# Grid2op/grid2op

Hardware: AMD Instinct MI355X
Metric: env steps/sec (batched DoNothing) (higher is better)
Workload: dtype f64; 1 GPU; l2rpn_case14_sandbox AC Newton-Raphson DoNothing env.step, batch=4096 lanes per GPU; env=l2rpn_case14_sandbox, lanes_per_gpu=4096, total_lanes=4096, env_steps_per_launch=16, observations=every env step -> HBM, cascade=False, kernels=grid-specialised at run time (gpf_jit_enable), parallelism=static lane shards x1, no collective

## Files before the change

### grid2op_amd/csrc/gridpf_sparse.hpp

```cpp
#pragma once
#include <type_traits>
#include "gridpf_common.hpp"

namespace gpf {

struct StatOff {
  int n_dbl, n_int;
  int n_int_hot;
  int br_y, br_bdc, sub_vn_kv, shunt_fact, gen_min_q, gen_max_q;
  int line_vn, load_vn, gen_vn, sto_vn, shunt_vn;
  int line_ka;
  int gen_qmin_tot, gen_qmax_tot;
  int gen_cnt;
  int dc_inv;
  int line_or_pos, line_ex_pos, line_or_sub, line_ex_sub, br_slot, gen_pos, gen_sub, gen_slack, load_pos, load_sub, sto_pos,
      sto_sub, shunt_sub, pair_rc, up, prog;
  int pos_line;
};
#define GPF_STATOFF_INTS(X) X(n_dbl) X(n_int) X(n_int_hot) X(br_y) X(br_bdc) X(sub_vn_kv) X(shunt_fact) X(gen_min_q) X(gen_max_q) X(line_vn) X(load_vn) \
  X(gen_vn) X(sto_vn) X(shunt_vn) X(line_ka) X(gen_qmin_tot) X(gen_qmax_tot) X(gen_cnt) X(dc_inv) X(line_or_pos) X(line_ex_pos) X(line_or_sub) \
  X(line_ex_sub) X(br_slot) X(gen_pos) X(gen_sub) X(gen_slack) X(load_pos) X(load_sub) X(sto_pos) X(sto_sub) X(shunt_sub) X(pair_rc) X(up) X(prog) X(pos_line)
static_assert(sizeof(StatOff) == sizeof(int) * (0 GPF_STATOFF_INTS(GPF_COUNT_FIELD)), "GPF_STATOFF_INTS must list every field of StatOff");
template <class T, bool IN_LDS>
struct SP {
// ... 1109 lines not shown
    if (PROG_LDS) return scalar_lu_flat<GW, true, false>(FL, sv.prog.p, c.A, c.A, tid, dbg);
    return scalar_lu_flat<GW, true, false>(FL, gptr(flat_g), c.A, c.A, tid, dbg);
  };
  if (!warm && !fuse_dc) {
#ifdef GPF_TIMING
    bool ok = dc_inv ? true : (NB == 1) ? lu_dc(&stamps.v[20])
                                        : lu_ac(&stamps.v[20]);
#else
    bool ok = dc_inv ? true : (NB == 1) ? lu_dc(nullptr) : lu_ac(nullptr);
#endif
    for (int i = tid; i < nbus; i += GW) {
      double th;
      if (dc_inv) {
        auto row_times_rhs = [&](const auto tab) -> double {
          double t0 = 0.0, t1 = 0.0;
          for (int k0 = 0; k0 < nbus; k0 += MVC) {
            double a_[MVC], r_[MVC];
#pragma unroll
            for (int q = 0; q < MVC; ++q) {
              const int k = k0 + q < nbus ? k0 + q : nbus - 1;
              a_[q] = tab[k * nbus + i];
              r_[q] = *rhsT(k);
            }
#pragma unroll
            for (int q = 0; q < MVC; q += 2) {
              if (k0 + q < nbus) t0 = fma(a_[q], r_[q], t0);
              if (k0 + q + 1 < nbus) t1 = fma(a_[q + 1], r_[q + 1], t1);
            }
          }
          return t0 + t1;
        };
        th = S.so.dc_inv >= 0 ? row_times_rhs(sv.dc_inv) : row_times_rhs(sv.dc_inv_g);
      } else if (NB == 1) {
        const double d = dc_kept ? c.Adc[i] : c.A[(size_t)i * 2];
        if (!(fabs(d) > 1e-300) || !(fabs(d) < 1e300)) ok = false;
        th = *rhsT(i) * fast_rcp(d);
      } else th = *rhsT(i);
      const int bt = c.btype[i];
      c.va[i] = (bt == BT_PQ || bt == BT_PV) ? th : 0.0;
      if (bt != BT_OFF && !(fabs(th) < 1e300)) ok = false;
    }
    if (NB == 1 && ctl.dcf && !dc_skip)
      for (int q = tid; q < S.nslot; q += GW) c.Adc[q] = c.A[(size_t)q * 2];
    GPF_LSYNC();
    if (WPI == 1 && dc_inv && G::block_any_u(ts.dc_out >= 0)) {
      const int lo_ = ts.dc_out >= 0 ? ts.dc_out : 0;
      const int f_ = sv.line_or_sub[lo_], t_ = sv.line_ex_sub[lo_];
      const double bl = ts.dc_out >= 0 ? sv.br_bdc[lo_] : 0.0;
      const bool f_ref = c.btype[f_] == BT_REF, t_ref = c.btype[t_] == BT_REF;
      const double dth = c.va[f_] - c.va[t_];
      const double xff = f_ref ? 0.0 : dcinv(f_ * nbus + f_), xtt = t_ref ? 0.0 : dcinv(t_ * nbus + t_);
      const double xft = (f_ref || t_ref) ? 0.0 : dcinv(t_ * nbus + f_);
      const double den = 1.0 - bl * (xff - 2.0 * xft + xtt);
      if (!(fabs(den) > 1e-12)) ok = false;
      const double kk = bl * dth / den;
      for (int i = tid; i < nbus; i += GW) {
        const int bt = c.btype[i];
        const double u_ = (f_ref ? 0.0 : dcinv(f_ * nbus + i)) - (t_ref ? 0.0 : dcinv(t_ * nbus + i));
        if (bt == BT_PQ || bt == BT_PV) c.va[i] += u_ * kk;
      }
      GPF_LSYNC();
    }
    if (status == 0 && G::any(!ok)) status = 4;
    if (G::block_all_u(status != 0)) return status;
  }
  GPF_STAMPS(4);

  int it = 0;
  if (!is_dc) {
    bool converged = false;
    bool done = status != 0;
    const int n_pairs = S.nslot_y * NB * NB;
    auto t_of = [&](const double2 y, double ei, double fi, double ej, double fj, double& tr_, double& ti_) {
      const double aa = y.x * ej - y.y * fj, bb = y.x * fj + y.y * ej;
      tr_ = ei * aa + fi * bb;
      ti_ = fi * aa - ei * bb;
    };
    if (nwr) {
      const bool p_on = tid < S.n_up, b_on = tid < nbus;
      const int ib = b_on ? tid : 0;
      const unsigned w0 = p_on ? (unsigned)sv.up[2 * tid] : 0u, w1 = p_on ? (unsigned)sv.up[2 * tid + 1] : 0u;
      const int u = (int)(w0 & 0xffffu), v = (int)(w0 >> 16), suv = (int)(w1 & 0xffffu), svu = (int)(w1 >> 16);
      constexpr bool KEEP_Y = IPW > 1;
      const double2* const p_yuv = reinterpret_cast<const double2*>(c.Yb + (size_t)suv * 2);
      const double2* const p_yvu = reinterpret_cast<const double2*>(c.Yb + (size_t)svu * 2);
      const double2* const p_yd = reinterpret_cast<const double2*>(c.Yb + (size_t)ib * 2);
      const double2 yuv0 = *p_yuv, yvu0 = *p_yvu, ydiag0 = *p_yd;
      const int btu = c.btype[u], btv = c.btype[v];
      const int bt = c.btype[ib];
      const double psp0 = c.Psp[ib], qsp0 = c.Qsp[ib];
#define NWR_YUV (KEEP_Y ? yuv0 : *p_yuv)
#define NWR_YVU (KEEP_Y ? yvu0 : *p_yvu)
#define NWR_YD (KEEP_Y ? ydiag0 : *p_yd)
#define NWR_PSP (KEEP_Y ? psp0 : c.Psp[ib])
#define NWR_QSP (KEEP_Y ? qsp0 : c.Qsp[ib])
      double va, vm;
#ifdef GPF_TIMING
      asm volatile("s_waitcnt lgkmcnt(0)" ::: "memory");
      GPF_STAMPS(20);
#endif
      if (fuse_dc) {
        const int vi = fast_pre ? c.vidx[ib] : -1;
        const double vm_lds = fast_pre ? 1.0 : c.vm[ib];
        if (b_on) c.ivm[ib] = psp0 - c.Gs[ib];
        GPF_LSYNC();
        auto row_times_rhs = [&](const auto tab, const bool by_row) -> double {
          double t0 = 0.0, t1 = 0.0;
          for (int k0 = 0; k0 < nbus; k0 += MVC) {
            double a_[MVC], r_[MVC];
#pragma unroll
            for (int q = 0; q < MVC; ++q) {
              const int k = k0 + q < nbus ? k0 + q : nbus - 1;
              a_[q] = by_row ? tab[ib * nbus + k] : tab[k * nbus + ib];
              r_[q] = c.ivm[k];
            }
#pragma unroll
            for (int q = 0; q < MVC; q += 2) {
              if (k0 + q < nbus) t0 = fma(a_[q], r_[q], t0);
              if (k0 + q + 1 < nbus) t1 = fma(a_[q + 1], r_[q + 1], t1);
            }
          }
          return t0 + t1;
        };
        const double th = S.so.dc_inv >= 0 ? row_times_rhs(sv.dc_inv, STAGE == 2) : row_times_rhs(sv.dc_inv_g, false);
        const bool live = (bt == BT_PQ || bt == BT_PV);
        va = live ? th : 0.0;
        vm = (vi >= 0 && (bt == BT_PV || bt == BT_REF)) ? GPF_INJ(oo.inj_gen_vm + vi) : vm_lds;
        const bool th_bad = b_on && bt != BT_OFF && !(fabs(th) < 1e300);
        if (status == 0 && G::any(th_bad)) { status = 4; done = true; }
      } else { va = c.va[ib]; vm = c.vm[ib]; }
#ifdef GPF_TIMING
      GPF_STAMPS(21);
#endif
      const bool act = p_on && (btu != BT_OFF) && (btv != BT_OFF);
      const bool uP = (btu == BT_PQ || btu == BT_PV), uQ = (btu == BT_PQ), vP = (btv == BT_PQ || btv == BT_PV), vQ = (btv == BT_PQ);
      const bool acc_u = act && (yuv0.x != 0.0 || yuv0.y != 0.0), acc_v = act && (yvu0.x != 0.0 || yvu0.y != 0.0);
      const bool rowP = (bt == BT_PQ || bt == BT_PV), rowQ = (bt == BT_PQ);
      const bool diag_on = bt != BT_OFF && (ydiag0.x != 0.0 || ydiag0.y != 0.0);
      double* const Ad0 = bel(ib, 0, 0);
      double* const Ad1 = bel(ib, 1, 0);
      double* const b_uv0 = bel(suv, 0, 0); double* const b_uv1 = bel(suv, 1, 0);
      double* const b_vu0 = bel(svu, 0, 0); double* const b_vu1 = bel(svu, 1, 0);
      double e, f, ivm, Sr = 0.0, Si = 0.0;
      {
        double sn_, co;
        fast_sincos(va, sn_, co);
        e = vm * co; f = vm * sn_; ivm = fast_rcp(vm);
        if (b_on) { setEF(ib, e, f); c.ivm[ib] = ivm; *SreP(ib) = 0.0; *SimP(ib) = 0.0; }
      }
      for (int i = S.nslot_y * 2 + tid; i < S.nslot * 2; i += GW) { c.A[i] = 0.0; c.A[HS + i] = 0.0; }
      GPF_LSYNC();
      GPF_STAMPS(10);
      asm volatile("; GPF_NEWTON_NWR_BEGIN" ::: "memory");
      while (true) {
        if (p_on) {
          const double2 efu = EF(u), efv = EF(v);
          const double ivmu = c.ivm[u], ivmv = c.ivm[v];
          double tr_, ti_, sr_, si_;
          const double2 yuv = NWR_YUV, yvu = NWR_YVU;
          t_of(yuv, efu.x, efu.y, efv.x, efv.y, tr_, ti_);
          t_of(yvu, efv.x, efv.y, efu.x, efu.y, sr_, si_);
          *reinterpret_cast<double2*>(b_uv0) = make_double2((uP && vP) ? ti_ : 0.0, (uP && vQ) ? tr_ * ivmv : 0.0);
          *reinterpret_cast<double2*>(b_uv1) = make_double2((uQ && vP) ? -tr_ : 0.0, (uQ && vQ) ? ti_ * ivmv : 0.0);
          *reinterpret_cast<double2*>(b_vu0) = make_double2((vP && uP) ? si_ : 0.0, (vP && uQ) ? sr_ * ivmu : 0.0);
          *reinterpret_cast<double2*>(b_vu1) = make_double2((vQ && uP) ? -sr_ : 0.0, (vQ && uQ) ? si_ * ivmu : 0.0);
          if (acc_u) { atomicAdd(SreP(u), tr_); atomicAdd(SimP(u), ti_); }
          if (acc_v) { atomicAdd(SreP(v), sr_); atomicAdd(SimP(v), si_); }
        }
        GPF_LSYNC();
        if (it == 0) GPF_STAMPS(11);
        double fabs_mis = 0.0;
        bool bad = false;
        if (b_on) {
          Sr = *SreP(ib); Si = *SimP(ib);
          const double2 ydiag = NWR_YD;
          const double psp = NWR_PSP, qsp = NWR_QSP;
          double tr_, ti_;
          t_of(ydiag, e, f, e, f, tr_, ti_);
          if (diag_on) { Sr += tr_; Si += ti_; }
          const double2 r0 = make_double2(rowP ? ti_ : 0.0, (rowP && rowQ) ? tr_ * ivm : 0.0);
          const double2 r1 = make_double2((rowQ && rowP) ? -tr_ : 0.0, rowQ ? ti_ * ivm : 0.0);
          *reinterpret_cast<double2*>(Ad0) = make_double2(rowP ? r0.x - Si : 1.0, rowQ ? fma(Sr, ivm, r0.y) : r0.y);
          *reinterpret_cast<double2*>(Ad1) = make_double2(rowQ ? r1.x + Sr : r1.x, rowQ ? fma(Si, ivm, r1.y) : 1.0);
          const double mp = rowP ? (Sr - psp) : 0.0;
          const double mq = rowQ ? (Si - qsp) : 0.0;
          *rhsT(ib) = -mp; *rhsV(ib) = -mq;
          const double am = fmax(fabs(mp), fabs(mq));
          if (!(am <= 1e300)) bad = true;
          fabs_mis = am;
        }
        if (!done) {
          const unsigned fl = G::template any2<0>(!(fabs_mis < tol_pu), bad);
          if (fl & 2u) { status = 1; done = true; }
          else if (!(fl & 1u)) { converged = true; done = true; }
          else if (it >= max_iter) done = true;
          else ++it;
        }
        if (G::block_all_u(done)) break;
        GPF_LSYNC();
        if (it == 1) GPF_STAMPS(12);
#ifdef GPF_TIMING
        const bool ok = lu_ac(it == 1 ? &stamps.v[32] : nullptr);
#else
        const bool ok = lu_ac(nullptr);
#endif
        if (it == 1) GPF_STAMPS(13);
        bool fin = true, piv_ok = true;
        if (b_on) {
          double2 dx = make_double2(*rhsT(ib), *rhsV(ib));
          const double2 dA = *reinterpret_cast<const double2*>(Ad0), dB = *reinterpret_cast<const double2*>(Ad1);
          const double det = fma(dA.x, dB.y, -dA.y * dB.x);
          if (!(fabs(det) > 1e-300) || !(fabs(det) < 1e300)) piv_ok = false;
          const double rd = fast_rcp(det);
          dx = make_double2(fma(dB.y, dx.x, -dA.y * dx.y) * rd, fma(dA.x, dx.y, -dB.x * dx.x) * rd);
          if (!done && bt != BT_OFF) {
            if (!(fabs(dx.x) < 1e300) || !(fabs(dx.y) < 1e300)) fin = false;
            if (bt == BT_PQ || bt == BT_PV) va += dx.x;
            if (bt == BT_PQ) vm += dx.y;
            if (vm < 0.0) { vm = -vm; va += 3.14159265358979323846; }
            if (fabs(va) > 3.14159265358979323846) va = remainder(va, 6.28318530717958647692);
          }
          double sn_, co;
          fast_sincos(va, sn_, co);
          e = vm * co; f = vm * sn_; ivm = fast_rcp(vm);
          setEF(ib, e, f);
          c.ivm[ib] = ivm;
          *SreP(ib) = 0.0;
          *SimP(ib) = 0.0;
        }
        for (int i = S.nslot_y * 2 + tid; i < S.nslot * 2; i += GW) { c.A[i] = 0.0; c.A[HS + i] = 0.0; }
        GPF_LSYNC();
        if (!done && G::template any2<1>(!ok || !piv_ok, !fin) != 0u) { status = 4; done = true; }
        if (it == 1) GPF_STAMPS(14);
        asm volatile("; GPF_NEWTON_NWR_BACKEDGE" ::: "memory");
      }
      if (b_on) { *SreP(ib) = Sr; *SimP(ib) = Si; c.va[ib] = va; c.vm[ib] = vm; }
#undef NWR_YUV
#undef NWR_YVU
#undef NWR_YD
#undef NWR_PSP
#undef NWR_QSP
    } else {
      for (int i = tid; i < nbus; i += GW) {
        const double va = c.va[i], vmi = c.vm[i];
        double sn_, co;
        fast_sincos(va, sn_, co);
        setEF(i, vmi * co, vmi * sn_);
        if (NB == 1) c.ivm[i] = fast_rcp(vmi);
        *SreP(i) = 0.0;
        *SimP(i) = 0.0;
        if (WPI > 1) { *rhsT(i) = 0.0; *rhsV(i) = 0.0; }
      }
      if (BS == 2) { for (int i = S.nslot_y * 2 + tid; i < S.nslot * 2; i += GW) { c.A[i] = 0.0; c.A[HS + i] = 0.0; } }
      else for (int i = S.nslot_y * B2 + tid; i < S.nslot_lu * B2; i += GW) c.A[i] = 0.0;
      GPF_LSYNC();
      GPF_STAMPS(10);
      unsigned rc_first = 0, rc_first1 = 0;
      if (STAGE == 0 && !YR) {
        if (NB == 1) { if (tid < S.n_up) { rc_first = (unsigned)sv.up[2 * tid]; rc_first1 = (unsigned)sv.up[2 * tid + 1]; } }
        else if (tid < n_pairs) rc_first = (unsigned)sv.pair_rc[tid / (NB * NB)];
      }
      while (true) {
        if (NB == 1) {
          auto upair_item = [&](const unsigned w0, const unsigned w1, const double2 yuv, const double2 yvu) {
            const int u = (int)(w0 & 0xffffu), v = (int)(w0 >> 16), suv = (int)(w1 & 0xffffu), svu = (int)(w1 >> 16);
            const int btu = c.btype[u], btv = c.btype[v];
            const double2 efu = EF(u), efv = EF(v);
            const double eu = efu.x, fu = efu.y, ivmu = c.ivm[u], ev = efv.x, fv = efv.y, ivmv = c.ivm[v];
            double tr_, ti_, sr_, si_;
            t_of(yuv, eu, fu, ev, fv, tr_, ti_);
            t_of(yvu, ev, fv, eu, fu, sr_, si_);
            const bool act = (btu != BT_OFF) && (btv != BT_OFF);
            const bool uP = (btu == BT_PQ || btu == BT_PV), uQ = (btu == BT_PQ), vP = (btv == BT_PQ || btv == BT_PV), vQ = (btv == BT_PQ);
            *reinterpret_cast<double2*>(bel(suv, 0, 0)) = make_double2((uP && vP) ? ti_ : 0.0, (uP && vQ) ? tr_ * ivmv : 0.0);
            *reinterpret_cast<double2*>(bel(suv, 1, 0)) = make_double2((uQ && vP) ? -tr_ : 0.0, (uQ && vQ) ? ti_ * ivmv : 0.0);
            *reinterpret_cast<double2*>(bel(svu, 0, 0)) = make_double2((vP && uP) ? si_ : 0.0, (vP && uQ) ? sr_ * ivmu : 0.0);
            *reinterpret_cast<double2*>(bel(svu, 1, 0)) = make_double2((vQ && uP) ? -sr_ : 0.0, (vQ && uQ) ? si_ * ivmu : 0.0);
            if (act && (yuv.x != 0.0 || yuv.y != 0.0)) { atomicAdd(wave1 ? rhsT(u) : SreP(u), tr_); atomicAdd(wave1 ? rhsV(u) : SimP(u), ti_); }
            if (act && (yvu.x != 0.0 || yvu.y != 0.0)) { atomicAdd(wave1 ? rhsT(v) : SreP(v), sr_); atomicAdd(wave1 ? rhsV(v) : SimP(v), si_); }
          };
          if (YR && S.n_up <= 2 * GW) {
            struct PairOps { int btu, btv; double2 efu, efv; double ivmu, ivmv; };
            auto pair_load = [&](const unsigned w0) -> PairOps {
              const int u = (int)(w0 & 0xffffu), v = (int)(w0 >> 16);
              PairOps o;
              o.btu = c.btype[u]; o.btv = c.btype[v]; o.efu = EF(u); o.efv = EF(v); o.ivmu = c.ivm[u]; o.ivmv = c.ivm[v];
              return o;
            };
            auto pair_fin = [&](const PairOps& o, const unsigned w0, const unsigned w1, const double2 yuv, const double2 yvu) {
              const int u = (int)(w0 & 0xffffu), v = (int)(w0 >> 16), suv = (int)(w1 & 0xffffu), svu = (int)(w1 >> 16);
              const int btu = o.btu, btv = o.btv;
              const double eu = o.efu.x, fu = o.efu.y, ivmu = o.ivmu, ev = o.efv.x, fv = o.efv.y, ivmv = o.ivmv;
              double tr_, ti_, sr_, si_;
              t_of(yuv, eu, fu, ev, fv, tr_, ti_);
              t_of(yvu, ev, fv, eu, fu, sr_, si_);
              const bool act = (btu != BT_OFF) && (btv != BT_OFF);
              const bool uP = (btu == BT_PQ || btu == BT_PV), uQ = (btu == BT_PQ), vP = (btv == BT_PQ || btv == BT_PV), vQ = (btv == BT_PQ);
              *reinterpret_cast<double2*>(bel(suv, 0, 0)) = make_double2((uP && vP) ? ti_ : 0.0, (uP && vQ) ? tr_ * ivmv : 0.0);
              *reinterpret_cast<double2*>(bel(suv, 1, 0)) = make_double2((uQ && vP) ? -tr_ : 0.0, (uQ && vQ) ? ti_ * ivmv : 0.0);
              *reinterpret_cast<double2*>(bel(svu, 0, 0)) = make_double2((vP && uP) ? si_ : 0.0, (vP && uQ) ? sr_ * ivmu : 0.0);
              *reinterpret_cast<double2*>(bel(svu, 1, 0)) = make_double2((vQ && uP) ? -sr_ : 0.0, (vQ && uQ) ? si_ * ivmu : 0.0);
              if (act && (yuv.x != 0.0 || yuv.y != 0.0)) { atomicAdd(wave1 ? rhsT(u) : SreP(u), tr_); atomicAdd(wave1 ? rhsV(u) : SimP(u), ti_); }
              if (act && (yvu.x != 0.0 || yvu.y != 0.0)) { atomicAdd(wave1 ? rhsT(v) : SreP(v), sr_); atomicAdd(wave1 ? rhsV(v) : SimP(v), si_); }
            };
            const bool on0 = tid < S.n_up, on1 = tid + GW < S.n_up;
            const PairOps o0 = pair_load(rcreg[0]), o1 = pair_load(rcreg[2]);
            if (on0) pair_fin(o0, rcreg[0], rcreg[1], yreg[0], yreg[1]);
            if (on1) pair_fin(o1, rcreg[2], rcreg[3], yreg[2], yreg[3]);
          } else if (YR) {
  #pragma unroll
            for (int k = 0; k < YR_PASSES; ++k) if (tid + k * GW < S.n_up) upair_item(rcreg[2 * k], rcreg[2 * k + 1], yreg[2 * k], yreg[2 * k + 1]);
          } else {
            unsigned p0 = rc_first, p1 = rc_first1;
            for (int k = tid; k < S.n_up; k += GW) {
              unsigned w0, w1;
              if (STAGE == 0) { w0 = p0; w1 = p1; if (k + GW < S.n_up) { p0 = (unsigned)sv.up[2 * (k + GW)]; p1 = (unsigned)sv.up[2 * (k + GW) + 1]; } }
              else { w0 = (unsigned)sv.up[2 * k]; w1 = (unsigned)sv.up[2 * k + 1]; }
              upair_item(w0, w1, *reinterpret_cast<const double2*>(c.Yb + (size_t)(w1 & 0xffffu) * 2),
                         *reinterpret_cast<const double2*>(c.Yb + (size_t)(w1 >> 16) * 2));
            }
          }
        } else {
          auto pair_item = [&](int pr, const double2 y, const unsigned rc) {
            const int slot = pr / (NB * NB), bi = (pr / NB) % NB, bj = pr % NB;
            const int si = (int)(rc & 0xffffu), sj = (int)(rc >> 16);
            const int i = si * NB + bi, j = sj * NB + bj;
            const int bti = c.btype[i], btj = c.btype[j];
            const double2 efi = EF(i), efj = EF(j);
            const double ei = efi.x, fi = efi.y, ej = efj.x, fj = efj.y, vmj = c.vm[j];
            double tr_, ti_;
            t_of(y, ei, fi, ej, fj, tr_, ti_);
            const bool act = (bti != BT_OFF) && (btj != BT_OFF);
            const bool rowP = (bti == BT_PQ || bti == BT_PV), rowQ = (bti == BT_PQ);
            const bool colT = (btj == BT_PQ || btj == BT_PV), colV = (btj == BT_PQ);
            const double ivmj = fast_rcp(vmj);
            *reinterpret_cast<double2*>(bel(slot, 2 * bi, 2 * bj)) = make_double2((rowP && colT) ? ti_ : 0.0, (rowP && colV) ? tr_ * ivmj : 0.0);
            *reinterpret_cast<double2*>(bel(slot, 2 * bi + 1, 2 * bj)) = make_double2((rowQ && colT) ? -tr_ : 0.0, (rowQ && colV) ? ti_ * ivmj : 0.0);
            if (act && (y.x != 0.0 || y.y != 0.0)) { atomicAdd(wave1 ? rhsT(i) : SreP(i), tr_); atomicAdd(wave1 ? rhsV(i) : SimP(i), ti_); }
          };
          unsigned rc_pf = rc_first;
          for (int pr = tid; pr < n_pairs; pr += GW) {
            unsigned rc;
            if (STAGE == 0) { rc = rc_pf; if (pr + GW < n_pairs) rc_pf = (unsigned)sv.pair_rc[(pr + GW) / (NB * NB)]; }
            else rc = (unsigned)sv.pair_rc[pr / (NB * NB)];
            pair_item(pr, *reinterpret_cast<const double2*>(c.Yb + (size_t)pr * 2), rc);
          }
        }
        GPF_LSYNC();
        if (it == 0) GPF_STAMPS(11);
        double fabs_mis = 0.0;
        bool bad = false;
        for (int i = tid; i < nbus; i += GW) {
          const int sub = (NB == 1) ? i : i / NB, bi = lidx(i);
          double* Ad0 = bel(sub, 2 * bi, 2 * bi);
          double* Ad1 = bel(sub, 2 * bi + 1, 2 * bi);
          const int bt = c.btype[i];
          double Sr = *SreP(i), Si = *SimP(i);
          if (WPI > 1) { Sr += *rhsT(i); Si += *rhsV(i); }
          const double vmi = c.vm[i], psp = c.Psp[i], qsp = c.Qsp[i];
          const bool rowP = (bt == BT_PQ || bt == BT_PV), rowQ = (bt == BT_PQ);
          const double ivmi = NB == 1 ? c.ivm[i] : fast_rcp(vmi);
          double2 r0, r1;
          if (NB == 1) {
            const double2 y = YR ? yreg[2 * YR_PASSES] : *reinterpret_cast<const double2*>(c.Yb + (size_t)i * 2);
            const double2 efi = EF(i);
            const double ei = efi.x, fi = efi.y;
            double tr_, ti_;
            t_of(y, ei, fi, ei, fi, tr_, ti_);
            if (bt != BT_OFF && (y.x != 0.0 || y.y != 0.0)) { Sr += tr_; Si += ti_; }
            *SreP(i) = Sr; *SimP(i) = Si;
            r0 = make_double2(rowP ? ti_ : 0.0, (rowP && rowQ) ? tr_ * ivmi : 0.0);
            r1 = make_double2((rowQ && rowP) ? -tr_ : 0.0, rowQ ? ti_ * ivmi : 0.0);
          } else { r0 = *reinterpret_cast<const double2*>(Ad0); r1 = *reinterpret_cast<const double2*>(Ad1); }
          *reinterpret_cast<double2*>(Ad0) = make_double2(rowP ? r0.x - Si : 1.0, rowQ ? fma(Sr, ivmi, r0.y) : r0.y);
          *reinterpret_cast<double2*>(Ad1) = make_double2(rowQ ? r1.x + Sr : r1.x, rowQ ? fma(Si, ivmi, r1.y) : 1.0);
          const double mp = rowP ? (Sr - psp) : 0.0;
          const double mq = rowQ ? (Si - qsp) : 0.0;
          if (BS == 2) { *rhsT(i) = -mp; *rhsV(i) = -mq; }
          else *reinterpret_cast<double2*>(c.rhs + (size_t)sub * BS + 2 * bi) = make_double2(-mp, -mq);
          const double am = fmax(fabs(mp), fabs(mq));
          if (!(am <= 1e300)) bad = true;
          fabs_mis = fmax(fabs_mis, am);
        }
        if (!done) {
          const unsigned fl = G::template any2<0>(!(fabs_mis < tol_pu), bad);
// ... 681 lines not shown
    if (tid < g.n_shunt) k_same = kt[g.dim_topo + tid] == gptr(b.shunt_bus)[(size_t)inst * g.n_shunt + tid];
    {
      const auto kd = (GPF_GLOBAL const double*)(kb + sa.keep.off_kd);
      const auto inj_now = gptr(b.inj) + (size_t)inst * g.n_inj + oo.inj_sh_p;
      const double a0_ = tid < 2 * g.n_shunt ? kd[tid] : 0.0, b0_ = tid < 2 * g.n_shunt ? inj_now[tid] : 0.0;
      const double a1_ = tid + GW < 2 * g.n_shunt ? kd[tid + GW] : 0.0, b1_ = tid + GW < 2 * g.n_shunt ? inj_now[tid + GW] : 0.0;
      k_same &= a0_ == b0_ && a1_ == b1_;
    }
    const auto km16 = (GPF_GLOBAL const v4i_*)(kb + sa.keep.off_m);
    const int n_ch = (sa.keep.n_m + 3) >> 2;
#pragma unroll
    for (int u = 0; u < KC; ++u) { const int ch = tid + u * GW; im[u] = ch < n_ch ? km16[ch] : v4i_{0, 0, 0, 0}; }
    const auto ky = (GPF_GLOBAL const v2d_*)(kb + sa.keep.off_y);
    auto ld2 = [&](int i_) { const v2d_ t_ = ky[i_]; return make_double2(t_.x, t_.y); };
    if (YR) {
#pragma unroll
      for (int k = 0; k < YR_PASSES; ++k) {
        const int pr = tid + k * GW;
        const bool on_ = pr < S.n_up;
        rcreg[2 * k] = on_ ? (unsigned)sv.up[2 * pr] : 0u; rcreg[2 * k + 1] = on_ ? (unsigned)sv.up[2 * pr + 1] : 0u;
        yreg[2 * k] = on_ ? ld2(2 * pr) : make_double2(0.0, 0.0);
        yreg[2 * k + 1] = on_ ? ld2(2 * pr + 1) : make_double2(0.0, 0.0);
      }
      yreg[2 * YR_PASSES] = tid < g.n_sub ? ld2(2 * S.n_up + tid) : make_double2(0.0, 0.0);
    } else {
#pragma unroll
      for (int u = 0; u < KY; ++u) { const int i = tid + u * GW; yy[u] = i < S.nslot_y ? ld2(i) : make_double2(0.0, 0.0); }
    }
    const auto ka = (GPF_GLOBAL const double*)(kb + sa.keep.off_d);
#pragma unroll
    for (int u = 0; u < KA; ++u) { const int q = tid + u * GW; aa[u] = (keep_dcf && q < S.nslot) ? ka[q] : 0.0; }
  }
  const int tab = b.lane_table ? gptr(b.lane_table)[inst] : 0;
  const int off = b.lane_offset ? gptr(b.lane_offset)[inst] : 0;
  int row = chron_row_index(sa.t, off, sa.T);
  const bool has_sc = b.lane_scale != nullptr;
  const bool has_delta = b.lane_gen_delta != nullptr;
  float sc_p0 = 1.f, sc_q0 = 1.f, gd0 = 0.f;
  if (has_sc && tid < g.n_load) { const auto sc = gptr(b.lane_scale) + (size_t)inst * 2 * g.n_load; sc_p0 = sc[tid]; sc_q0 = sc[g.n_load + tid]; }
  if (has_delta && tid < g.n_gen) gd0 = gptr(b.lane_gen_delta)[(size_t)inst * g.n_gen + tid];
  if (STAGE) { const auto inj_g = gptr(b.inj) + (size_t)inst * g.n_inj; for (int i = oo.inj_sto_p + tid; i < g.n_inj; i += GW) c.inj[i] = inj_g[i]; }
  TopoState ts;
  ts.status = 0; ts.nb = 0; ts.dc_base = false; ts.dc_out = -1; ts.gen_base = false; ts.tc[0] = ts.tc[1] = -1;
  bool reuse = false;
  int n_iter = 0, nb = 0, st = 0, rounds = 0;
  float lim_first = 1e30f, lim_second = 1e30f;
  int ovc_first = 0, inc_first = 0, ovc_second = 0;
  if (tid < g.n_line) { lim_first = gptr(b.thermal_limit)[tid]; ovc_first = gptr(b.overflow_count)[(size_t)inst * g.n_line + tid]; }
  const bool regs2 = g.n_line <= 2 * GW;
  if (regs2 && tid + GW < g.n_line) { lim_second = gptr(b.thermal_limit)[tid + GW]; ovc_second = gptr(b.overflow_count)[(size_t)inst * g.n_line + tid + GW]; }
  int ep_steps = 0, ep_resets = 0;
  if (tid == 0 && !ghost) { ep_steps = gptr(b.episode)[2 * (size_t)inst]; ep_resets = gptr(b.episode)[2 * (size_t)inst + 1]; }
  constexpr int LWE = GW < WAVE ? GW : WAVE;
  constexpr bool env_on = ENV && NB == 1;
  EnvRegs er;
  er.target = er.actual = er.prev_p = er.charge = er.amount_prev = er.curt_prev = 0.f; er.limit = 1.f; er.already = false; er.fresh = true;
  er.illegal = 0;
  float env_ar0 = 0.f, env_as0 = 0.f, env_ac0 = -1.f;
  if (env_on && tid < LWE) {
    const EnvDyn& E = P->env;
    if (tid < g.n_gen) {
      const size_t q = (size_t)inst * g.n_gen + tid;
      er.target = gptr(E.target)[q]; er.actual = gptr(E.actual)[q]; er.prev_p = gptr(E.prev_p)[q]; er.already = gptr(E.already)[q] != 0;
      if (E.act_redisp) env_ar0 = gptr(E.act_redisp)[q];
      er.limit = gptr(E.limit)[q];
      if (E.act_curtail) env_ac0 = gptr(E.act_curtail)[q];
    }
    if (tid < g.n_sto) {
      er.charge = gptr(E.charge)[(size_t)inst * g.n_sto + tid];
      if (E.act_storage) env_as0 = gptr(E.act_storage)[(size_t)inst * g.n_sto + tid];
    }
    er.amount_prev = gptr(E.amount_prev)[inst];
    er.curt_prev = gptr(E.curt_prev)[inst];
    er.fresh = gptr(E.fresh)[inst] != 0;
    er.illegal = gptr(E.illegal)[inst];
  }
  bool env_fail = false;
  constexpr bool PF9 = WPI == 1;
  float pf_lp = 0.f, pf_lq = 0.f, pf_pp = 0.f, pf_pv = 1.f;
  if (PF9) {
    const auto ch0 = gptr(b.chron) + ((size_t)tab * sa.T + row) * g.n_chron;
    if (tid < g.n_load) { pf_lp = ch0[tid]; pf_lq = ch0[g.n_load + tid]; }
    if (tid < g.n_gen) { pf_pp = ch0[2 * g.n_load + tid]; pf_pv = ch0[2 * g.n_load + g.n_gen + tid]; }
  }
  bool keep_hit = false, keep_dirty = false;
  bool keep_claim = false;
  GPF_STAMPS(34);
  if (keep_on) {
    const auto kb = (GPF_GLOBAL const unsigned char*)sa.keep.p + (YR ? (size_t)sa.keep.stride : 0);
    const auto kt = (GPF_GLOBAL const int*)kb + KEEP_HDR_INTS;
    bool same = k_same;
#pragma unroll
    for (int u = 0; u < KT; ++u) same &= kk[u] == tn[u];
    {
      const auto topo_now = gptr(b.topo) + (size_t)inst * g.dim_topo;
      const auto shb_now = gptr(b.shunt_bus) + (size_t)inst * g.n_shunt;
      const auto kd = (GPF_GLOBAL const double*)(kb + sa.keep.off_kd);
      const auto inj_now = gptr(b.inj) + (size_t)inst * g.n_inj + oo.inj_sh_p;
      for (int i = tid + KT * GW; i < g.dim_topo; i += GW) same &= kt[i] == topo_now[i];
      for (int i = tid + GW; i < g.n_shunt; i += GW) same &= kt[g.dim_topo + i] == shb_now[i];
      for (int i = tid + 2 * GW; i < 2 * g.n_shunt; i += GW) same &= kd[i] == inj_now[i];
    }
    GPF_STAMPS(36);
    const bool valid = k_h0 > KEEP_VALID && k_h0 - KEEP_VALID < sa.keep.launch;
    {
      const auto km16 = (GPF_GLOBAL const v4i_*)(kb + sa.keep.off_m);
      const auto ky = (GPF_GLOBAL const v2d_*)(kb + sa.keep.off_y);
      const auto ka = (GPF_GLOBAL const double*)(kb + sa.keep.off_d);
      int* const img = c.btype;
      v2i_* const img2 = reinterpret_cast<v2i_*>(img);
      const int n_m = sa.keep.n_m;
      auto put4 = [&](int ch, const v4i_ t_) {
        if (4 * ch + 3 < n_m) { img2[2 * ch] = v2i_{t_.x, t_.y}; img2[2 * ch + 1] = v2i_{t_.z, t_.w}; }
        else { if (4 * ch < n_m) img[4 * ch] = t_.x; if (4 * ch + 1 < n_m) img[4 * ch + 1] = t_.y; if (4 * ch + 2 < n_m) img[4 * ch + 2] = t_.z; }
      };
      const int n_ch = (n_m + 3) >> 2;
#pragma unroll
      for (int u = 0; u < KC; ++u) { const int ch = tid + u * GW; if (ch < n_ch) put4(ch, im[u]); }
      for (int ch = tid + KC * GW; ch < n_ch; ch += GW) put4(ch, km16[ch]);
      if (!YR) {
        double2* const yl = reinterpret_cast<double2*>(c.Yb);
#pragma unroll
        for (int u = 0; u < KY; ++u) { const int i = tid + u * GW; if (i < S.nslot_y) yl[i] = yy[u]; }
        for (int i = tid + KY * GW; i < S.nslot_y; i += GW) { const v2d_ t_ = ky[i]; yl[i] = make_double2(t_.x, t_.y); }
      }
      if (keep_dcf && (k_h2 & 4)) {
#pragma unroll
        for (int u = 0; u < KA; ++u) { const int q = tid + u * GW; if (q < S.nslot) c.Adc[q] = aa[u]; }
        for (int q = tid + KA * GW; q < S.nslot; q += GW) c.Adc[q] = ka[q];
      }
    }
    GPF_STAMPS(37);
    const unsigned hb = G::template any_bits<3, 4>(((same && valid) ? 0u : 1u) | ((k_h2 & 1) ? 0u : 2u) | ((k_h2 & 4) ? 0u : 4u) | (same ? 0u : 8u));
    const unsigned hbb = IPW == 1 ? hb : ((__any(hb & 1u) ? 1u : 0u) | (__any(hb & 2u) ? 2u : 0u) | (__any(hb & 4u) ? 4u : 0u));
    keep_hit = !(hbb & 1u) && (!keep_dcf || !(hbb & 2u) || !(hbb & 4u));
    keep_claim = !(hb & 8u) && k_h0 == KEEP_KEYED && !ghost;
    if (keep_hit) {
      ts.status = k_h1 & 0xff; ts.nb = k_h1 >> 8; ts.dc_base = (k_h2 & 1) != 0; ts.gen_base = (k_h2 & 2) != 0; ts.dc_out = (k_h2 >> 3) - 1;
      reuse = true;
    }
    GPF_STAMPS(38);
    GPF_LSYNC();
  }
  GPF_STAMPS(39);
#define GPF_REDERIVE()                                                                                              \
  do {                                                                                                              \
    grp = grp0; tid = tid0; inst = inst0;                                                                           \
    asm volatile("" : "+v"(grp), "+v"(tid), "+v"(inst));                                                            \
    carve_sparse<NB>(c, smem + (size_t)grp * per_inst, g, lds_nslot, lds_nslot_y, STAGE != 0, lds_rows, lds_dcf);   \
  } while (0)
  const bool tobs = b.traj_out != nullptr;
  FlatWords<flat_words_ct<NB, IPW, WPI>()> FW;
  flat_words_load<GW>(FW, FL, gptr(S.flat[GWI]), tid0);
  for (int step = 0; step < sa.n_steps; ++step) {
    GPF_REDERIVE();
    const bool last = step + 1 == sa.n_steps;
    const bool otraj = tobs && step < b.traj_cap;
    int orow = otraj ? step * (int)b.lane_stride + inst : inst;
    GPF_STAMPS(19);
    bool sums_in_k9 = false, skip_inj = false;
    float k9_lp0 = 0.f, k9_lq0 = 0.f, k9_lp1 = 0.f, k9_lq1 = 0.f, k9_pp = 0.f, k9_vm = 1.f;
    {
      const auto ch = gptr(b.chron) + ((size_t)tab * sa.T + row) * g.n_chron;
      const auto sc = gptr(b.lane_scale) + (size_t)inst * 2 * g.n_load;
      const auto gdelta = gptr(b.lane_gen_delta) + (size_t)inst * g.n_gen;
      const auto inj_g = gptr(b.inj) + (size_t)inst * g.n_inj;
      bool any_maint = false;
      const auto mrow = gptr(b.maint) + ((size_t)tab * sa.T + row) * g.n_line;
      if (b.maint) {
        const auto topo = gptr(b.topo) + (size_t)inst * g.dim_topo;
        bool hit = false;
        if (!ghost)
        for (int l = tid; l < g.n_line; l += GW)
          if (mrow[l] && topo[sv.line_or_pos[l]] != -1) { topo[sv.line_or_pos[l]] = -1; topo[sv.line_ex_pos[l]] = -1; hit = true; }
        any_maint = G::block_any(hit);
        if (any_maint) reuse = false;
      }
      if (!reuse) { const auto topo = gptr(b.topo) + (size_t)inst * g.dim_topo; for (int i = tid; i < g.dim_topo; i += GW) c.topo[i] = topo[i]; }
      if (any_maint) {
        GPF_SYNC();
        for (int l = tid; l < g.n_line; l += GW) if (mrow[l]) { c.topo[sv.line_or_pos[l]] = -1; c.topo[sv.line_ex_pos[l]] = -1; }
      }
      float pp_pre = pf_pp, pv_pre = pf_pv, lp_pre = pf_lp, lq_pre = pf_lq;
      constexpr bool PRE2 = WPI > 1;
      constexpr int gw9 = WPI > 1 ? WAVE : GW;
      float lp2 = 0.f, lq2 = 0.f, sc2p = 1.f, sc2q = 1.f;
      if (!PF9) {
        pp_pre = tid < g.n_gen ? ch[2 * g.n_load + tid] : 0.f;
        pv_pre = tid < g.n_gen ? ch[2 * g.n_load + g.n_gen + tid] : 1.f;
        if (PRE2 && tid < gw9) {
          if (tid < g.n_load) { lp_pre = ch[tid]; lq_pre = ch[g.n_load + tid]; }
          if (tid + gw9 < g.n_load) {
            lp2 = ch[tid + gw9]; lq2 = ch[g.n_load + tid + gw9];
            if (has_sc) { sc2p = sc[tid + gw9]; sc2q = sc[g.n_load + tid + gw9]; }
          }
        }
      }
      if (PF9 && !last) {
        const int row_n = row + 1 >= sa.T ? 0 : row + 1;
        const auto chn = gptr(b.chron) + ((size_t)tab * sa.T + row_n) * g.n_chron;
        if (tid < g.n_load) { pf_lp = chn[tid]; pf_lq = chn[g.n_load + tid]; }
        if (tid < g.n_gen) { pf_pp = chn[2 * g.n_load + tid]; pf_pv = chn[2 * g.n_load + g.n_gen + tid]; }
      }
      double sum_load = 0.0, sum_prod = 0.0;
      sums_in_k9 = reuse;
      skip_inj = WPI > 1 && !STAGE && sums_in_k9 && !last && !env_on && sa.cascade == 0 && g.n_load <= 2 * WAVE && g.n_gen <= WAVE;
      const double inv_sn9 = g.inv_sn_mva;
      if (sums_in_k9) {
        const int nbus9 = TC ? S.n : g.n_sub * NB;
        for (int i = tid; i < nbus9; i += GW) { c.Psp[i] = 0.0; c.Qsp[i] = 0.0; c.Gs[i] = 0.0; }
        GPF_LSYNC();
      }
      GPF_STAMPS(16);
      const bool lane9 = tid < gw9;
      if (lane9)
      for (int i = tid; i < g.n_load; i += gw9) {
        const bool i0_ = (PF9 || PRE2) && i == tid, i1_ = PRE2 && i == tid + gw9;
        float lp = i0_ ? lp_pre : i1_ ? lp2 : ch[i], lq = i0_ ? lq_pre : i1_ ? lq2 : ch[g.n_load + i];
        if (has_sc) { lp *= (i == tid) ? sc_p0 : i1_ ? sc2p : sc[i]; lq *= (i == tid) ? sc_q0 : i1_ ? sc2q : sc[g.n_load + i]; }
        if (STAGE) { c.inj[oo.inj_load_p + i] = (double)lp; c.inj[oo.inj_load_q + i] = (double)lq; }
        else if (!skip_inj) { inj_g[oo.inj_load_p + i] = (double)lp; inj_g[oo.inj_load_q + i] = (double)lq; }
        if (i == tid) { k9_lp0 = lp; k9_lq0 = lq; } else if (i1_) { k9_lp1 = lp; k9_lq1 = lq; }
        sum_load += (double)lp;
        if (sums_in_k9) {
          const int bu = c.load_b[i];
          if (bu >= 0) { atomicAdd(&c.Psp[bu], -(double)lp * inv_sn9); atomicAdd(&c.Qsp[bu], -(double)lq * inv_sn9); }
        }
      }
      if (lane9)
      for (int i = tid; i < g.n_gen; i += gw9)
        if (!sv.gen_slack[i]) sum_prod += (double)(i == tid ? pp_pre : ch[2 * g.n_load + i]);
      float scale_p = 1.0f;
      GPF_STAMPS(17);
      if (sa.rebalance_on) {
        G::template sum2<0>(sum_load, sum_prod);
        scale_p = (sum_prod > 0.0) ? (float)(sa.rebalance * sum_load / sum_prod) : 1.0f;
      }
      GPF_STAMPS(18);
      env_fail = false;
      float env_np = 0.f;
      if (env_on && (WPI == 1 || tid < WAVE)) {
        float np_k = tid < g.n_gen ? pp_pre : 0.f;
        if (tid < g.n_gen && !sv.gen_slack[tid]) np_k *= scale_p;
        float sto_pw = 0.f;
        const bool ok_e = env_dynamics_step<LWE>(P->env, tid, g.n_gen, g.n_sto, np_k, step == 0 ? env_ar0 : 0.f,
                                                 (step == 0 || P->env.hold_storage) ? env_as0 : 0.f, step == 0 ? env_ac0 : -1.f, er, sto_pw);
        env_fail = !ok_e;
        env_np = np_k;
        if (tid < g.n_sto) {
          if (STAGE) c.inj[oo.inj_sto_p + tid] = (double)sto_pw;
          else inj_g[oo.inj_sto_p + tid] = (double)sto_pw;
        }
      }
      if (lane9)
      for (int i = tid; i < g.n_gen; i += gw9) {
        float pp = (i == tid) ? pp_pre : ch[2 * g.n_load + i];
        if (!sv.gen_slack[i]) pp *= scale_p;
        if (env_on) pp = env_np + er.actual;
        if (has_delta) pp += (i == tid) ? gd0 : gdelta[i];
        const float pv_kv = (i == tid) ? pv_pre : ch[2 * g.n_load + g.n_gen + i];
        const float vn = (float)sv.gen_vn[i];
        const double vm_pu = (double)(pv_kv / vn);
        if (STAGE) { c.inj[oo.inj_gen_p + i] = (double)pp; c.inj[oo.inj_gen_vm + i] = vm_pu; }
        else if (!skip_inj) { inj_g[oo.inj_gen_p + i] = (double)pp; inj_g[oo.inj_gen_vm + i] = vm_pu; }
        if (i == tid) { k9_pp = pp; k9_vm = pv_kv / vn; }
        if (sums_in_k9) {
          const int bu = c.gen_b[i];
          if (bu >= 0 && !sv.gen_slack[i]) atomicAdd(&c.Psp[bu], (double)pp * inv_sn9);
        }
      }
      GPF_STAMPS(29);
      if (sums_in_k9 && lane9) {
        for (int i = tid; i < g.n_sto; i += gw9) {
          const int bu = c.sto_b[i];
          if (bu >= 0) {
            const double sp = STAGE ? c.inj[oo.inj_sto_p + i] : (double)inj_g[oo.inj_sto_p + i];
            const double sq = STAGE ? c.inj[oo.inj_sto_q + i] : (double)inj_g[oo.inj_sto_q + i];
            atomicAdd(&c.Psp[bu], -sp * inv_sn9);
            atomicAdd(&c.Qsp[bu], -sq * inv_sn9);
          }
        }
        for (int i = tid; i < g.n_shunt; i += gw9) {
          const int bu = c.sh_b[i];
          if (bu >= 0) {
            const double hp = STAGE ? c.inj[oo.inj_sh_p + i] : (double)inj_g[oo.inj_sh_p + i];
            atomicAdd(&c.Gs[bu], hp * sv.shunt_fact[i] * inv_sn9);
          }
        }
      }
      GPF_SYNC_IF(!STAGE && !skip_inj);
      GPF_STAMPS(30);
    }
    n_iter = 0; nb = 0; st = 0; rounds = 0;
    float a_first = 0.f;
    {
      const auto dround = gptr(b.disc_round) + (size_t)inst * g.n_line;
      for (int l = tid; l < g.n_line; l += GW) dround[l] = -1;
      const auto inc_flag = (GPF_GLOBAL int*)(gptr(b.rho) + (size_t)inst * g.n_line);
      if (sa.cascade) for (int l = tid + GW; l < g.n_line; l += GW) inc_flag[l] = 0;
      inc_first = 0;
    }
    if (!reuse) keep_dirty = true;
    bool more = true;
    bool first = true;
    bool tripped = false;
    while (true) {
      GPF_REDERIVE();
      int it_k = 0, nb_k = 0;
      SolveCtl ctl;
      ctl.inj_staged = true; ctl.topo_staged = first; ctl.reuse = first && reuse; ctl.dcf = P->dcf != 0 && (sa.n_steps > 1 || keep_on); ctl.write_bus = last; ctl.warm = sa.warm_start != 0 && !(keep_hit && step == 0); ctl.sums_done = first && sums_in_k9;
      orow = otraj ? step * (int)b.lane_stride + inst : inst;
      ctl.otraj = otraj; ctl.orow = orow; ctl.write_topo = otraj || (keep_hit && step == 0);
      ctl.tc_rebuild = keep_hit && step == 0;
      ctl.inj_regs = skip_inj; ctl.r_lp0 = k9_lp0; ctl.r_lq0 = k9_lq0; ctl.r_lp1 = k9_lp1; ctl.r_lq1 = k9_lq1; ctl.r_pp = k9_pp; ctl.r_vm = k9_vm;
      GPF_STAMPS(31);
      const int st_k = solve_instance_sparse<NB, STAGE, IPW, WPI, TC, YR>(P, S, FL, sv, c, yreg, rcreg, FW, inst, sa.is_dc, max_iter, tol_pu, tid, ctl, ts, it_k, nb_k, a_first GPF_STAMPS_ARG);
      first = false;
      GPF_SYNC_IF(sa.cascade != 0 && g.n_line > GW);
      if (more) { st = st_k; n_iter = it_k; nb = nb_k; }
      if (st != 0 || !sa.cascade || rounds >= sa.max_rounds) more = false;
      int any_disc = 0;
      if (more && !ghost) {
        const auto out = gptr(otraj ? b.traj_out : b.out) + (size_t)orow * g.n_out;
        const auto ovc = gptr(b.overflow_count) + (size_t)inst * g.n_line;
        const auto dround = gptr(b.disc_round) + (size_t)inst * g.n_line;
        const auto inc_flag = (GPF_GLOBAL int*)(gptr(b.rho) + (size_t)inst * g.n_line);
        const auto topo = gptr(b.topo) + (size_t)inst * g.dim_topo;
        const auto thermal_limit = gptr(b.thermal_limit);
        for (int l = tid; l < g.n_line; l += GW) {
          const bool own = l == tid, own2 = regs2 && l == tid + GW;
          const float a = own ? a_first : (c.out_l ? c.out_l[oo.a_or + l] : (float)out[oo.a_or + l]);
          const float lim = own ? lim_first : own2 ? lim_second : (float)thermal_limit[l];
          const bool on = c.lor_b[l] >= 0;
          bool disc = on && (a > sa.hard_overflow * lim);
          int inc = own ? inc_first : (int)inc_flag[l];
          if (on && (a > sa.soft_overflow * lim) && !inc) { inc = 1; if (own) inc_first = 1; else inc_flag[l] = 1; }
          if (on && ((own ? ovc_first : own2 ? ovc_second : (int)ovc[l]) + inc) > sa.nb_ts_allowed) disc = true;
          if (disc) {
            topo[sv.line_or_pos[l]] = -1;
            topo[sv.line_ex_pos[l]] = -1;
            dround[l] = rounds;
            any_disc = 1;
          }
        }
      }
      const bool anyd = more && G::any(any_disc);
      GPF_SYNC_IF(G::block_any_u(anyd));
      if (more && !anyd) more = false;
      if (more) tripped = true;
      if (!G::block_any_u(more)) break;
      if (more) ++rounds;
    }
    GPF_STAMPS(9);
    GPF_REDERIVE();
    if (env_on) {
      const bool ef = WPI > 1 ? (__syncthreads_or(env_fail) != 0) : env_fail;
      if (ef && st == 0) st = 6;
    }
    orow = otraj ? step * (int)b.lane_stride + inst : inst;
    if (st != 0) { write_nan_results<GW>(g, b, inst, tid, orow, otraj); a_first = __builtin_nanf(""); }
    GPF_SYNC_IF(G::block_any_u(st != 0));
    {
      const auto out = gptr(otraj ? b.traj_out : b.out) + (size_t)orow * g.n_out;
      const auto ovc = gptr(b.overflow_count) + (size_t)inst * g.n_line;
      const auto rho = gptr(b.rho) + (size_t)inst * g.n_line;
      const auto thermal_limit = gptr(b.thermal_limit);
      GPF_GLOBAL float* traj = nullptr;
      if (b.traj_rho && step < b.traj_cap) traj = gptr(b.traj_rho) + ((size_t)step * b.lane_stride + inst) * g.n_line;
      for (int l = tid; l < g.n_line; l += GW) {
        const bool own = l == tid, own2 = regs2 && l == tid + GW;
        const float lim = own ? lim_first : own2 ? lim_second : (float)thermal_limit[l];
        const float a = own ? a_first : ((st == 0 && c.out_l) ? c.out_l[oo.a_or + l] : (float)out[oo.a_or + l]);
        const float r_ = a / lim;
        if (!traj || last || sa.cascade) rho[l] = r_;
        if (traj) traj[l] = r_;
        if (!ghost) {
          const int prev = own ? ovc_first : own2 ? ovc_second : (int)ovc[l];
          const int now = (a > sa.soft_overflow * lim) ? prev + 1 : 0;
          if (own) ovc_first = now; else if (own2) ovc_second = now;
          if (!regs2 || last) ovc[l] = now;
        }
      }
      if (sa.nb_ts_reco >= 0 && st == 0 && !ghost) {
        const auto cool = gptr(b.cooldown) + (size_t)inst * g.n_line;
        const auto dround = gptr(b.disc_round) + (size_t)inst * g.n_line;
        const auto mdur = gptr(b.maint_dur) + ((size_t)tab * sa.T + row) * g.n_line;
        GPF_GLOBAL short* tcool = nullptr;
        if (b.traj_cool && step < b.traj_cap) tcool = gptr(b.traj_cool) + ((size_t)step * b.lane_stride + inst) * g.n_line;
        for (int l = tid; l < g.n_line; l += GW) {
          int cd = cool[l];
          cd = cd > 0 ? cd - 1 : 0;
          if (dround[l] >= 0) cd = sa.nb_ts_reco;
          if (b.maint_dur) { const int md = (int)mdur[l]; cd = md > cd ? md : cd; }
          cool[l] = cd;
          if (tcool) tcool[l] = (short)(cd > 32767 ? 32767 : cd);
        }
      }
    }
    const bool failed = st != 0;
    if (tid == 0) {
      const auto s = gptr(b.status) + (size_t)inst * 4;
      s[0] = st; s[1] = n_iter; s[2] = nb; s[3] = rounds;
      if (!ghost) {
        gptr(b.done)[inst] = failed ? 1 : 0;
        if (b.traj_status && step < b.traj_cap) gptr(b.traj_status)[(size_t)step * b.lane_stride + inst] = (signed char)st;
        if (failed) { if (sa.auto_reset) { ep_steps = 0; ++ep_resets; } } else ++ep_steps;
      }
    }
    if (failed && sa.auto_reset && !ghost) {
      const auto t0 = gptr(b.topo0) + (size_t)inst * g.dim_topo;
      const auto topo = gptr(b.topo) + (size_t)inst * g.dim_topo;
      const auto ovc = gptr(b.overflow_count) + (size_t)inst * g.n_line;
      for (int i = tid; i < g.dim_topo; i += GW) topo[i] = t0[i];
      for (int l = tid; l < g.n_line; l += GW) ovc[l] = 0;
      if (sa.nb_ts_reco >= 0) { const auto cool = gptr(b.cooldown) + (size_t)inst * g.n_line; for (int l = tid; l < g.n_line; l += GW) cool[l] = 0; }
      ovc_first = 0; ovc_second = 0;
      if (env_on) {
        er.target = er.actual = er.prev_p = er.amount_prev = er.curt_prev = 0.f; er.limit = 1.f; er.already = false; er.fresh = true;
        er.illegal = 0;
        er.charge = (tid < g.n_sto && P->env.charge0) ? gptr(P->env.charge0)[tid] : 0.f;
      }
    }
    reuse = !G::block_any_u(failed || tripped);
    GPF_STAMPS(7);
    if (++row >= sa.T) row = 0;
    if (!last) GPF_SYNC_IF(G::block_any_u(failed && sa.auto_reset != 0));
  }
#undef GPF_REDERIVE
  grp = grp0; tid = tid0; inst = inst0;
  if (keep_on) {
    const auto kb = (GPF_GLOBAL unsigned char*)sa.keep.p + (YR ? (size_t)sa.keep.stride : 0);
    const auto hdr = (GPF_GLOBAL int*)kb;
    bool won = false;
    if (keep_claim && reuse && keep_dirty && tid == 0) won = atomicCAS((int*)hdr, KEEP_KEYED, KEEP_CLAIMED) == KEEP_KEYED;
    const bool all_dcb = G::block_all_u(ts.dc_base);
    if (G::any(won)) {
      typedef double v2d_ __attribute__((ext_vector_type(2)));
      const auto km = (GPF_GLOBAL int*)(kb + sa.keep.off_m);
      const int* const img = c.btype;
      for (int i = tid; i < sa.keep.n_m; i += GW) km[i] = img[i];
      const auto ky = (GPF_GLOBAL v2d_*)(kb + sa.keep.off_y);
      auto st2 = [&](int i_, const double2 v_) { v2d_ t_; t_.x = v_.x; t_.y = v_.y; ky[i_] = t_; };
      if (YR) {
#pragma unroll
        for (int k = 0; k < YR_PASSES; ++k) {
          const int pr = tid + k * GW;
          if (pr < S.n_up) { st2(2 * pr, yreg[2 * k]); st2(2 * pr + 1, yreg[2 * k + 1]); }
        }
        if (tid < g.n_sub) st2(2 * S.n_up + tid, yreg[2 * YR_PASSES]);
      } else {
        const double2* const yl = reinterpret_cast<const double2*>(c.Yb);
        for (int i = tid; i < S.nslot_y; i += GW) st2(i, yl[i]);
      }
      const bool adc = keep_dcf && !all_dcb;
      if (adc) { const auto ka = (GPF_GLOBAL double*)(kb + sa.keep.off_d); for (int q = tid; q < S.nslot; q += GW) ka[q] = c.Adc[q]; }
      if (tid == 0) {
        hdr[1] = (ts.status & 0xff) | (ts.nb << 8);
        hdr[2] = (ts.dc_base ? 1 : 0) | (ts.gen_base ? 2 : 0) | (adc ? 4 : 0) | ((ts.dc_out + 1) << 3);
        hdr[0] = KEEP_VALID + sa.keep.launch;
      }
    }
  }
  if (tobs) {
    const int ls = sa.n_steps <= b.traj_cap ? sa.n_steps - 1 : b.traj_cap - 1;
    const size_t r = (size_t)ls * b.lane_stride + inst;
    GPF_SYNC();
    { const auto s_ = gptr(b.traj_out) + r * g.n_out; const auto d_ = gptr(b.out) + (size_t)inst * g.n_out; for (int i = tid; i < g.n_out; i += GW) d_[i] = s_[i]; }
    { const auto s_ = gptr(b.traj_topo) + r * g.dim_topo; const auto d_ = gptr(b.topo_out) + (size_t)inst * g.dim_topo; for (int i = tid; i < g.dim_topo; i += GW) d_[i] = s_[i]; }
    { const auto s_ = gptr(b.traj_shb) + r * g.n_shunt; const auto d_ = gptr(b.shunt_bus_out) + (size_t)inst * g.n_shunt; for (int i = tid; i < g.n_shunt; i += GW) d_[i] = s_[i]; }
    { const auto s_ = gptr(b.traj_lstat) + r * g.n_line; const auto d_ = gptr(b.line_status) + (size_t)inst * g.n_line; for (int i = tid; i < g.n_line; i += GW) d_[i] = s_[i]; }
  }
  if (tid == 0 && !ghost) { gptr(b.episode)[2 * (size_t)inst] = ep_steps; gptr(b.episode)[2 * (size_t)inst + 1] = ep_resets; }
  if (STAGE && !ghost) {
    const auto inj_g = gptr(b.inj) + (size_t)inst * g.n_inj;
    const int n_wb = env_on ? oo.inj_sto_q : oo.inj_sto_p;
    for (int i = tid; i < n_wb; i += GW) inj_g[i] = c.inj[i];
  }
  if (env_on && tid < LWE && !ghost) {
    const EnvDyn& E = P->env;
    if (tid < g.n_gen) {
      const size_t q = (size_t)inst * g.n_gen + tid;
      gptr(E.target)[q] = er.target; gptr(E.actual)[q] = er.actual; gptr(E.prev_p)[q] = er.prev_p; gptr(E.already)[q] = er.already ? 1 : 0;
      gptr(E.limit)[q] = er.limit;
    }
    if (tid < g.n_sto) gptr(E.charge)[(size_t)inst * g.n_sto + tid] = er.charge;
    if (tid == 0) {
      gptr(E.amount_prev)[inst] = er.amount_prev; gptr(E.curt_prev)[inst] = er.curt_prev; gptr(E.fresh)[inst] = er.fresh ? 1 : 0;
      gptr(E.illegal)[inst] = er.illegal;
    }
  }
  GPF_STAMPS(15);
  GPF_STAMPS_FLUSH(inst);
}

}
```

Baseline: 210.7 million env steps/sec.

## Merge Newton update-failure vote into convergence ballot and cache storage/shunt sums in registers

The Newton loop now folds the post-LU pivot and finiteness checks into the next iteration's convergence ballot, which removes one wave-wide vote per iteration. It also computes the diagonal-term products before the LDS barrier and clears the A fill slots before the update step. Separately, for single-warp, multi-instance configurations it keeps the storage and shunt bus contributions in registers across env steps, skips re-clearing the disc_round array every step when there is no cascade, and reads the DC-flag from an LDS copy. These changes cut per-iteration sync and per-step global traffic, at the cost of more register pressure and a one-iteration delay in reporting an update failure.

Result: no change. 211.1 million env steps/sec, median of 5 (+0.2%).

```diff
diff --git a/grid2op_amd/csrc/gridpf_sparse.hpp b/grid2op_amd/csrc/gridpf_sparse.hpp
--- a/grid2op_amd/csrc/gridpf_sparse.hpp
+++ b/grid2op_amd/csrc/gridpf_sparse.hpp
@@ -1285,6 +1285,7 @@
       GPF_LSYNC();
       GPF_STAMPS(10);
       asm volatile("; GPF_NEWTON_NWR_BEGIN" ::: "memory");
+      bool upd_fail = false, upd_nonfin = false;
       while (true) {
         if (p_on) {
           const double2 efu = EF(u), efv = EF(v);
@@ -1300,19 +1301,22 @@
           if (acc_u) { atomicAdd(SreP(u), tr_); atomicAdd(SimP(u), ti_); }
           if (acc_v) { atomicAdd(SreP(v), sr_); atomicAdd(SimP(v), si_); }
         }
+        double tr_ = 0.0, ti_ = 0.0;
+        double2 r0 = make_double2(0.0, 0.0), r1 = make_double2(0.0, 0.0);
+        if (b_on) {
+          const double2 ydiag = NWR_YD;
+          t_of(ydiag, e, f, e, f, tr_, ti_);
+          r0 = make_double2(rowP ? ti_ : 0.0, (rowP && rowQ) ? tr_ * ivm : 0.0);
+          r1 = make_double2((rowQ && rowP) ? -tr_ : 0.0, rowQ ? ti_ * ivm : 0.0);
+        }
         GPF_LSYNC();
         if (it == 0) GPF_STAMPS(11);
         double fabs_mis = 0.0;
         bool bad = false;
         if (b_on) {
           Sr = *SreP(ib); Si = *SimP(ib);
-          const double2 ydiag = NWR_YD;
           const double psp = NWR_PSP, qsp = NWR_QSP;
-          double tr_, ti_;
-          t_of(ydiag, e, f, e, f, tr_, ti_);
           if (diag_on) { Sr += tr_; Si += ti_; }
-          const double2 r0 = make_double2(rowP ? ti_ : 0.0, (rowP && rowQ) ? tr_ * ivm : 0.0);
-          const double2 r1 = make_double2((rowQ && rowP) ? -tr_ : 0.0, rowQ ? ti_ * ivm : 0.0);
           *reinterpret_cast<double2*>(Ad0) = make_double2(rowP ? r0.x - Si : 1.0, rowQ ? fma(Sr, ivm, r0.y) : r0.y);
           *reinterpret_cast<double2*>(Ad1) = make_double2(rowQ ? r1.x + Sr : r1.x, rowQ ? fma(Si, ivm, r1.y) : 1.0);
           const double mp = rowP ? (Sr - psp) : 0.0;
@@ -1323,8 +1327,9 @@
           fabs_mis = am;
         }
         if (!done) {
-          const unsigned fl = G::template any2<0>(!(fabs_mis < tol_pu), bad);
-          if (fl & 2u) { status = 1; done = true; }
+          const unsigned fl = G::template any_bits<0, 4>((!(fabs_mis < tol_pu) ? 1u : 0u) | (bad ? 2u : 0u) | (upd_fail ? 4u : 0u) | (upd_nonfin ? 8u : 0u));
+          if (fl & 12u) { status = 4; done = true; }
+          else if (fl & 2u) { status = 1; done = true; }
           else if (!(fl & 1u)) { converged = true; done = true; }
           else if (it >= max_iter) done = true;
           else ++it;
@@ -1338,6 +1343,7 @@
         const bool ok = lu_ac(nullptr);
 #endif
         if (it == 1) GPF_STAMPS(13);
+        for (int i = S.nslot_y * 2 + tid; i < S.nslot * 2; i += GW) { c.A[i] = 0.0; c.A[HS + i] = 0.0; }
         bool fin = true, piv_ok = true;
         if (b_on) {
           double2 dx = make_double2(*rhsT(ib), *rhsV(ib));
@@ -1361,9 +1367,8 @@
           *SreP(ib) = 0.0;
           *SimP(ib) = 0.0;
         }
-        for (int i = S.nslot_y * 2 + tid; i < S.nslot * 2; i += GW) { c.A[i] = 0.0; c.A[HS + i] = 0.0; }
+        upd_fail = !ok || !piv_ok; upd_nonfin = !fin;
         GPF_LSYNC();
-        if (!done && G::template any2<1>(!ok || !piv_ok, !fin) != 0u) { status = 4; done = true; }
         if (it == 1) GPF_STAMPS(14);
         asm volatile("; GPF_NEWTON_NWR_BACKEDGE" ::: "memory");
       }
@@ -2351,6 +2356,12 @@
   const bool tobs = b.traj_out != nullptr;
   FlatWords<flat_words_ct<NB, IPW, WPI>()> FW;
   flat_words_load<GW>(FW, FL, gptr(S.flat[GWI]), tid0);
+  constexpr bool W1 = WPI == 1;
+  constexpr bool SS_REGS = W1 && IPW > 1 && !env_on;
+  const bool ss_fit = SS_REGS && g.n_sto <= GW && g.n_shunt <= GW;
+  bool ss_held = false;
+  int ss_sto_b = -1, ss_sh_b = -1;
+  double ss_sto_p = 0.0, ss_sto_q = 0.0, ss_sh_g = 0.0;
   for (int step = 0; step < sa.n_steps; ++step) {
     GPF_REDERIVE();
     const bool last = step + 1 == sa.n_steps;
@@ -2469,6 +2480,28 @@
         }
       }
       GPF_STAMPS(29);
+      if (SS_REGS && ss_fit && sums_in_k9 && lane9) {
+        if (!ss_held) {
+          ss_sto_b = -1; ss_sh_b = -1;
+          if (tid < g.n_sto) {
+            const int bu = c.sto_b[tid];
+            if (bu >= 0) {
+              const double sp = STAGE ? c.inj[oo.inj_sto_p + tid] : (double)inj_g[oo.inj_sto_p + tid];
+              const double sq = STAGE ? c.inj[oo.inj_sto_q + tid] : (double)inj_g[oo.inj_sto_q + tid];
+              ss_sto_b = bu; ss_sto_p = -sp * inv_sn9; ss_sto_q = -sq * inv_sn9;
+            }
+          }
+          if (tid < g.n_shunt) {
+            const int bu = c.sh_b[tid];
+            if (bu >= 0) {
+              const double hp = STAGE ? c.inj[oo.inj_sh_p + tid] : (double)inj_g[oo.inj_sh_p + tid];
+              ss_sh_b = bu; ss_sh_g = hp * sv.shunt_fact[tid] * inv_sn9;
+            }
+          }
+        }
+        if (ss_sto_b >= 0) { atomicAdd(&c.Psp[ss_sto_b], ss_sto_p); atomicAdd(&c.Qsp[ss_sto_b], ss_sto_q); }
+        if (ss_sh_b >= 0) atomicAdd(&c.Gs[ss_sh_b], ss_sh_g);
+      } else
       if (sums_in_k9 && lane9) {
         for (int i = tid; i < g.n_sto; i += gw9) {
           const int bu = c.sto_b[i];
@@ -2487,6 +2520,7 @@
           }
         }
       }
+      if (SS_REGS) ss_held = ss_fit && sums_in_k9;
       GPF_SYNC_IF(!STAGE && !skip_inj);
       GPF_STAMPS(30);
     }
@@ -2494,7 +2528,7 @@
     float a_first = 0.f;
     {
       const auto dround = gptr(b.disc_round) + (size_t)inst * g.n_line;
-      for (int l = tid; l < g.n_line; l += GW) dround[l] = -1;
+      if (!W1 || step == 0 || sa.cascade) for (int l = tid; l < g.n_line; l += GW) dround[l] = -1;
       const auto inc_flag = (GPF_GLOBAL int*)(gptr(b.rho) + (size_t)inst * g.n_line);
       if (sa.cascade) for (int l = tid + GW; l < g.n_line; l += GW) inc_flag[l] = 0;
       inc_first = 0;
@@ -2507,7 +2541,7 @@
       GPF_REDERIVE();
       int it_k = 0, nb_k = 0;
       SolveCtl ctl;
-      ctl.inj_staged = true; ctl.topo_staged = first; ctl.reuse = first && reuse; ctl.dcf = P->dcf != 0 && (sa.n_steps > 1 || keep_on); ctl.write_bus = last; ctl.warm = sa.warm_start != 0 && !(keep_hit && step == 0); ctl.sums_done = first && sums_in_k9;
+      ctl.inj_staged = true; ctl.topo_staged = first; ctl.reuse = first && reuse; ctl.dcf = (W1 ? lds_dcf : P->dcf != 0) && (sa.n_steps > 1 || keep_on); ctl.write_bus = last; ctl.warm = sa.warm_start != 0 && !(keep_hit && step == 0); ctl.sums_done = first && sums_in_k9;
       orow = otraj ? step * (int)b.lane_stride + inst : inst;
       ctl.otraj = otraj; ctl.orow = orow; ctl.write_topo = otraj || (keep_hit && step == 0);
       ctl.tc_rebuild = keep_hit && step == 0;
@@ -2589,7 +2623,7 @@
         for (int l = tid; l < g.n_line; l += GW) {
           int cd = cool[l];
           cd = cd > 0 ? cd - 1 : 0;
-          if (dround[l] >= 0) cd = sa.nb_ts_reco;
+          if ((!W1 || sa.cascade) && dround[l] >= 0) cd = sa.nb_ts_reco;
           if (b.maint_dur) { const int md = (int)mdur[l]; cd = md > cd ? md : cd; }
           cool[l] = cd;
           if (tcool) tcool[l] = (short)(cd > 32767 ? 32767 : cd);
```
